# Chris10M/Ev2Hands

Measured on AMD Instinct MI355X. Metric: event-windows/sec at B=256 N=2048 (f16x2), higher is better.
Workload: dtype f32 (each f32 operand split into 2 fp16 planes with per-window power-of-two range scaling, 3 plane products per MAC on the f16 MFMA, f32 accumulate); 1 GPU; TEHNet.forward+MANO both hands, B=256/GPU N=2048 C=4 fp32, E-clouds, random-init 342-key checkpoint, synthetic MANO-shaped assets; global_batch=256, points=2048, channels=4, precision=f16x2, forwards_in_flight=1, world_size_seen=1, parallelism=batch-shard x1

## Files before the change

ev2hands_amd/csrc/forward.hip:

```cpp
#include <cstdarg>
#include <cstdio>
#include <cstdlib>
#include <cstring>

#include "common.hpp"
#include "planes.hpp"
#include "ev2hands_hip.h"
#include "side_stream.hpp"
#include "workspace.hpp"

int ev2h_gemm_init();

static thread_local char g_err[512] = "";

void ev2h_set_error(const char* fmt, ...) {
    va_list ap;
    va_start(ap, fmt);
    vsnprintf(g_err, sizeof(g_err), fmt, ap);
    va_end(ap);
}

extern "C" const char* ev2h_last_error(void) { return g_err; }
extern "C" int ev2h_abi_version(void) { return EV2H_ABI_VERSION; }

// ... 107 lines not shown
    do {                          \
        int rc__ = (expr);        \
        if (rc__) return rc__;    \
    } while (0)

struct DenseOpt {
    const float* group_bias = nullptr; int group_rows = 0, ldbias = 0;
    int taps = 1, rows_per_seq = 0;
    int rowmax_rows = 0;
    int skinny = 0;
    int fam = EV2H_FAM_DENSE;
};

static ev2h_gemm_desc dense_desc(const Call& cx, const ev2h_dense& w, const float* X, int ldx, int M, float* Y, int ldy, int relu, const Rng& rg,
                                 const DenseOpt& o = {}) {
    ev2h_gemm_desc d{};
    d.skinny = o.skinny;
    d.x_amax = rg.xa; d.x_amax2 = rg.xa2; d.x_group_rows = rg.xg; d.y_amax = rg.ya; d.y_group_rows = rg.yg;
    d.X = X; d.ldx = ldx; d.W = w.W; d.ldw = w.ldw; d.Y = Y; d.ldy = ldy;
    d.M = M; d.N = w.O; d.K = w.K;
    d.bias = o.group_bias ? o.group_bias : w.b;
    d.bias_group_rows = o.group_rows; d.ldbias = o.ldbias;
    d.relu = relu; d.post_scale = w.post_scale; d.post_shift = w.post_shift;
    d.taps = o.taps; d.rows_per_seq = o.rows_per_seq; d.rowmax_rows = o.rowmax_rows;
    d.precision = cx.fam_prec(o.fam);
    d.Ws = (cx.prec != EV2H_PREC_F32) ? w.Ws : nullptr;
    d.ws_tile_rows = w.ws_tile_rows;
    d.w_unscale = w.w_unscale;
    return d;
}

static int dense(const Call& cx, const ev2h_dense& w, const float* X, int ldx, int M, float* Y, int ldy, int relu, ev2h_stream_t st, const Rng& rg,
                 const DenseOpt& o = {}) {
    const ev2h_gemm_desc d = dense_desc(cx, w, X, ldx, M, Y, ldy, relu, rg, o);
    return ev2h_gemm(&d, st);
}

static int sa_table(int precision, const ev2h_sa_module& m, const float* feat, int ldf, int B, int Npts, float* P1, ev2h_stream_t st,
                    const uint32_t* feat_amax, uint32_t* p1_amax, float* p1_scale, bool chain = true) {
    int c1sum = 0;
    float extra = 0.f;
    for (int i = 0; i < m.nbranch; ++i) {
        c1sum += m.br[i].C1;
        extra = fmaxf(extra, m.br[i].w1x_norm * (float)m.br[i].radius * 1.0000002f);
    }
    ev2h_gemm_desc g{};
    g.X = feat; g.ldx = ldf; g.W = m.W1f; g.ldw = m.kf; g.Y = P1; g.ldy = c1sum;
    g.M = B * Npts; g.N = c1sum; g.K = m.kf; g.bias = m.b1; g.taps = 1;
    g.precision = precision;
    g.w_unscale = m.w1f_unscale;
    if (precision != EV2H_PREC_F32 && m.W1fs) { g.Ws = m.W1fs; g.ws_tile_rows = 128; }
    if (feat_amax) {
        g.x_amax = feat_amax; g.x_group_rows = Npts;
        g.y_amax = p1_amax; g.y_group_rows = Npts;
        g.y_scale = p1_scale; g.y_bound_w = m.w1f_norm; g.y_bound_b = m.b1_max + extra;
        if (precision == EV2H_PREC_F16 && chain) {
            float wmul = 1.f, badd = g.y_bound_b;
            for (int i = 0; i < m.nbranch; ++i) {
                const float iu = 1.000001f / (m.br[i].w2_unscale > 0.f ? m.br[i].w2_unscale : 1.f);
                wmul = fmaxf(wmul, m.br[i].w2_norm * iu);
                badd = fmaxf(badd, (m.br[i].w2_norm * g.y_bound_b + m.br[i].b2_max) * iu);
            }
            g.y_bound_w *= wmul; g.y_bound_b = badd;
        }
    }
    return ev2h_gemm(&g, st);
}

static bool bf16_direct_layer1(int precision, const ev2h_sa_module& m) {
    static const bool table = getenv("EV2H_L1_TABLE") != nullptr;
    return precision != EV2H_PREC_F32 && m.kf == 8 && !table;
}

static int sa_branches(int precision, const char* tag, const ev2h_sa_module& m, const float* pts4, const float* ctr4, int32_t* const* gidx,
                       const int32_t* cnt, int B, int Npts, const float* P1, float* out, int ldo, ev2h_stream_t st, bool ranges,
                       const uint32_t* p1_amax, const float* p1_scale, uint32_t* out_amax, const float* feat = nullptr, int nfeat = 0,
                       const uint32_t* feat_amax = nullptr, float* xyz_out = nullptr, int xyz_ld = 0, int s_off = 0, int s_cnt = 0) {
    int c1sum = 0;
    for (int i = 0; i < m.nbranch; ++i) c1sum += m.br[i].C1;
    int coff1 = 0, coff3 = 0;
    for (int i = 0; i < m.nbranch; ++i) {
        const ev2h_sa_branch& br = m.br[i];
        ev2h_sa_desc d{};
        d.P1 = P1 + coff1; d.ldp = c1sum; d.pts4 = pts4; d.ctr4 = ctr4; d.gidx = gidx[i];
        d.W1x = br.W1x; d.W2 = br.W2; d.b2 = br.b2; d.W3 = br.W3; d.b3 = br.b3;
        d.out = out + coff3; d.ldo = ldo;
        d.B = B; d.Npts = Npts; d.S = m.npoint; d.K = br.K; d.C1 = br.C1; d.C2 = br.C2; d.C3 = br.C3;
        if (s_cnt > 0) { d.S = s_cnt; d.S_total = m.npoint; d.s_off = s_off; }
        d.precision = precision; d.W2s = br.W2s; d.W3s = br.W3s; d.w2_unscale = br.w2_unscale; d.w3_unscale = br.w3_unscale;
        const bool direct = feat && bf16_direct_layer1(precision, m);
        if (direct) {
            d.feat = feat; d.ldf = 8; d.W1f = m.W1f + (size_t)coff1 * m.kf; d.ldw1f = m.kf; d.b1 = m.b1 + coff1; d.nfeat = nfeat;
            d.w1f_unscale = br.w1f_unscale; d.w1x_unscale = br.w1x_unscale;
            if (ranges) { d.feat_amax = feat_amax; d.w1f_norm = m.w1f_norm; d.b1_max = m.b1_max; }
        }
        if (ranges) {
            if (!direct) { d.p1_scale = p1_scale; d.p1_amax = p1_amax; }
            d.out_amax = out_amax;
            d.w1x_norm = br.w1x_norm; d.dmax = (float)br.radius * 1.0000002f ; d.w2_norm = br.w2_norm; d.b2_max = br.b2_max;
        }
        d.cnt = cnt ? cnt + i : nullptr; d.cnt_ld = m.nbranch;
        if (i == 0 && xyz_out) { d.xyz_out = xyz_out; d.xyz_ld = xyz_ld; }
        char t[40];
        snprintf(t, sizeof(t), "%s.%d", tag, i);
        prof_begin(t, st);
        RUN(ev2h_sa_mlp_max(&d, st));
        prof_end(t, st);
        coff1 += br.C1;
        coff3 += br.C3;
    }
    return EV2H_OK;
}

static int sa_module(int precision, const char* tag, const ev2h_sa_module& m, const float* feat, int ldf, const float* pts4, const float* ctr4,
                     int32_t* const* gidx, const int32_t* cnt, int B, int Npts, float* P1, float* out, int ldo, ev2h_stream_t st,
                     const uint32_t* feat_amax, uint32_t* p1_amax, float* p1_scale, uint32_t* out_amax, int nfeat = 0, float* xyz_out = nullptr,
                     int xyz_ld = 0) {
    if (!bf16_direct_layer1(precision, m)) RUN(sa_table(precision, m, feat, ldf, B, Npts, P1, st, feat_amax, p1_amax, p1_scale));
    return sa_branches(precision, tag, m, pts4, ctr4, gidx, cnt, B, Npts, P1, out, ldo, st, feat_amax != nullptr, p1_amax, p1_scale, out_amax,
                       ldf == 8 ? feat : nullptr, nfeat, feat_amax, xyz_out, xyz_ld);
}

}

static int forward_body(const ev2h_weights* w, const ev2h_mano_consts* const* mano, float* xyz_cm, int B, int C, int N, int mhlnes,
                        const int64_t* fps_init, const ev2h_outputs* out, const Call& cx, bool* forked) {
    const Ws& ws = cx.ws;
    const ev2h_stream_t st = cx.st;
    const int R = B * N;
    const int prec = cx.prec;
    const int prec_sa = cx.fam_prec(EV2H_FAM_SA), prec_rows = cx.fam_prec(EV2H_FAM_ROWS), prec_q = cx.fam_prec(EV2H_FAM_QCONV);
    auto rg = [&](int xid, int xg, int yid = -1, int yg = 0, int xid2 = -1) {
        Rng r{};
        if (ws.ranges_on) {
            r.xa = ws.r(xid); r.xg = xg;
            if (xid2 >= 0) r.xa2 = ws.r(xid2);
            if (yid >= 0) { r.ya = ws.r(yid); r.yg = yg; }
        }
        return r;
    };
    if (ws.ranges_on) EV2H_CHECK_HIP(hipMemsetAsync(ws.i(WS_RANGES), 0, ws.L.count[WS_RANGES] * 4, (hipStream_t)st));

    RUN(ev2h_prep_points(xyz_cm, B, C, N, mhlnes, ws.f(WS_PTS4), ws.f(WS_FEAT8), ws.r(R_FEAT), st));
    const bool fork = cx.side != nullptr;
    const ev2h_stream_t sd = fork ? (ev2h_stream_t)cx.side->stream : st;
    RUN(cx.signal_side(EV_INPUT));
    *forked = fork;
    if (!bf16_direct_layer1(prec, w->sa1)) RUN(sa_table(prec_sa, w->sa1, ws.f(WS_FEAT8), 8, B, N, ws.f(WS_P1A), sd, ws.r(R_FEAT), ws.r(R_P1A), ws.p1scale(0)));
    RUN(cx.side_records(EV_SA1_TABLE));
    static const int chunk_env = [] { const char* e = getenv("EV2H_FPS_CHUNKS"); return e ? atoi(e) : -1; }();
    const int chunk_max_wg = chunk_env > 1 ? chunk_env : (N <= 2048 ? 0x7fffffff : 256), chunk_min_b = chunk_env > 1 ? 1 : 8;
    const bool chunked = fork && chunk_env != 0 && B >= chunk_min_b && 3 * B <= chunk_max_wg && bf16_direct_layer1(prec, w->sa1) && w->sa1.npoint % FPS_CHUNKS == 0;
    const bool side_queries = chunked && B >= 64 && N <= 2048;
    int32_t* gi1[3] = {ws.i(WS_GIDX1_0), ws.i(WS_GIDX1_1), ws.i(WS_GIDX1_2)};
    double rad1[3]; int ns1[3];
    for (int i = 0; i < 3; ++i) { rad1[i] = w->sa1.br[i].radius; ns1[i] = w->sa1.br[i].K; }
    const int S[3] = {512, 128, 128};
    const int64_t* init[3] = {fps_init, fps_init + 2 * (size_t)B, fps_init + 3 * (size_t)B};
    int32_t* idx[3] = {ws.i(WS_FPS1), ws.i(WS_FPSM_L), ws.i(WS_FPSM_R)};
    float* ctr[3] = {ws.f(WS_CTR1), ws.f(WS_CTRM_L), ws.f(WS_CTRM_R)};
    static const bool unfused_fp1 = getenv("EV2H_FP1_UNFUSED") != nullptr;
    const bool fp1_fused = prec != EV2H_PREC_F32 && w->fp1m.W1fs && !unfused_fp1;
    auto late_selections = [&](bool with_samplings) -> int {
        if (fp1_fused) {
            RUN(ev2h_three_nn_interp(ws.f(WS_PTS4), ws.f(WS_CTR1), B, N, 512, nullptr, 0, 0, nullptr, 0, ws.i(WS_NN1_IDX), ws.f(WS_NN1_W), nullptr, sd));
            RUN(cx.side_records(EV_FP1_NN));
        }
        if (with_samplings) RUN(ev2h_fps_multi(ws.f(WS_PTS4), B, N, 2, S + 1, init + 1, idx + 1, ctr + 1, sd));
        for (int h = 0; h < 2; ++h) {
            const ev2h_sa_module& m = w->mano_sa1[h];
            double rad[2]; int ns[2];
            int32_t* gi[2] = {ws.i(hand(WS_GIDXM0_L, h)), ws.i(hand(WS_GIDXM1_L, h))};
            for (int i = 0; i < 2; ++i) { rad[i] = m.br[i].radius; ns[i] = m.br[i].K; }
            RUN(ev2h_ball_query(ws.f(WS_PTS4), ws.f(hand(WS_CTRM_L, h)), B, N, 128, 2, rad, ns, gi, ws.i(hand(WS_CNTM_L, h)), sd));
        }
        return cx.side_records(EV_HAND_QUERIES);
    };
    if (!chunked) {
        RUN(ev2h_fps_multi(ws.f(WS_PTS4), B, N, 3, S, init, idx, ctr, st));
    } else {
        const int q = w->sa1.npoint / FPS_CHUNKS;
        for (int c = 0; c < FPS_CHUNKS; ++c) {
            RUN(ev2h_fps_multi_chunk(ws.f(WS_PTS4), B, N, side_queries ? 1 : 3, S, init, idx, ctr, c * q, (c + 1) * q, ws.f(WS_FPS_STATE), sd));
            if (side_queries) RUN(ev2h_ball_query_range(ws.f(WS_PTS4), ws.f(WS_CTR1), B, N, 512, c * q, q, 3, rad1, ns1, gi1, ws.i(WS_CNT1), sd));
            RUN(cx.side_records(EV_SA1_QUARTER0 + c));
        }
    }
    if (!chunked) RUN(cx.signal_side(EV_SAMPLED));
    int32_t* gi2[2] = {ws.i(WS_GIDX2_0), ws.i(WS_GIDX2_1)};
    {
        const ev2h_sa_module& m = w->sa2;
        RUN(ev2h_fps(ws.f(WS_CTR1), B, 512, 128, fps_init + (size_t)B, ws.i(WS_FPS2), ws.f(WS_CTR2), sd));
        double rad[2]; int ns[2];
        for (int i = 0; i < 2; ++i) { rad[i] = m.br[i].radius; ns[i] = m.br[i].K; }
        RUN(ev2h_ball_query(ws.f(WS_CTR1), ws.f(WS_CTR2), B, 512, 128, 2, rad, ns, gi2, ws.i(WS_CNT2), sd));
        RUN(cx.side_records(EV_SA2_QUERY));
    }
    if (!side_queries) RUN(late_selections(false));
    {
        const ev2h_sa_module& m = w->sa1;
        if (!chunked) {
            RUN(ev2h_ball_query(ws.f(WS_PTS4), ws.f(WS_CTR1), B, N, 512, 3, rad1, ns1, gi1, ws.i(WS_CNT1), st));
            RUN(cx.wait_side(EV_SA1_TABLE));
            RUN(sa_branches(prec_sa, "sa1", m, ws.f(WS_PTS4), ws.f(WS_CTR1), gi1, ws.i(WS_CNT1), B, N, ws.f(WS_P1A), ws.f(WS_L1CAT), 576, st, ws.ranges_on,
                            ws.r(R_P1A), ws.p1scale(0), ws.r(R_L1A), ws.f(WS_FEAT8), C, ws.r(R_FEAT)));
        } else {
            const int q = m.npoint / FPS_CHUNKS;
            for (int c = 0; c < FPS_CHUNKS; ++c) {
                RUN(cx.wait_side(EV_SA1_QUARTER0 + c));
                if (!side_queries) RUN(ev2h_ball_query_range(ws.f(WS_PTS4), ws.f(WS_CTR1), B, N, 512, c * q, q, 3, rad1, ns1, gi1, ws.i(WS_CNT1), st));
                RUN(sa_branches(prec_sa, "sa1", m, ws.f(WS_PTS4), ws.f(WS_CTR1), gi1, ws.i(WS_CNT1), B, N, ws.f(WS_P1A), ws.f(WS_L1CAT), 576, st, ws.ranges_on,
                                ws.r(R_P1A), ws.p1scale(0), ws.r(R_L1A), ws.f(WS_FEAT8), C, ws.r(R_FEAT), nullptr, 0, c * q, q));
            }
        }
    }
    {
        const ev2h_sa_module& m = w->sa2;
        RUN(cx.wait_side(EV_SA2_QUERY));
        RUN(sa_module(prec_sa, "sa2", m, ws.f(WS_L1CAT), 576, ws.f(WS_CTR1), ws.f(WS_CTR2), gi2, ws.i(WS_CNT2), B, 512, ws.f(WS_P1B), ws.f(WS_L2BUF), 520, st,
                      ws.r(R_L1A), ws.r(R_P1B), ws.p1scale(1), ws.r(R_L2), 0, ws.f(WS_L2BUF) + 512, 520));
    }
    RUN(dense(cx, w->sa3[0], ws.f(WS_L2BUF), 520, B * 128, ws.f(WS_SA3H1), 256, 1, st, rg(R_L2, 128, R_SA3H1, 128, R_FEAT)));
    RUN(dense(cx, w->sa3[1], ws.f(WS_SA3H1), 256, B * 128, ws.f(WS_SA3H2), 512, 1, st, rg(R_SA3H1, 128, R_SA3H2, 128)));
    RUN(dense(cx, w->sa3[2], ws.f(WS_SA3H2), 512, B * 128, ws.f(WS_L3), 1024, 1, st, rg(R_SA3H2, 128, R_L3, 1), {.rowmax_rows = 128}));
    RUN(dense(cx, w->fp3_bcast, ws.f(WS_L3), 1024, B, ws.f(WS_FP3BIAS), 256, 0, st, rg(R_L3, 1), {.skinny = 1}));
    if (side_queries) {
        RUN(cx.signal_side(EV_ENC_SA3));
        RUN(late_selections(true));
    }
    RUN(dense(cx, w->fp3_skip, ws.f(WS_L2BUF), 520, B * 128, ws.f(WS_FP3H), 256, 1, st, rg(R_L2, 128, R_FP3H, 128, R_FEAT),
              {.group_bias = ws.f(WS_FP3BIAS), .group_rows = 128, .ldbias = 256}));
    RUN(dense(cx, w->fp3_1, ws.f(WS_FP3H), 256, B * 128, ws.f(WS_FP3O), 256, 1, st, rg(R_FP3H, 128, R_FP3O, 128)));
    RUN(ev2h_three_nn_interp(ws.f(WS_CTR1), ws.f(WS_CTR2), B, 512, 128, ws.f(WS_FP3O), 256, 256, ws.f(WS_L1CAT) + 320, 576,
                             ws.i(WS_NN2_IDX), ws.f(WS_NN2_W), ws.r(R_L1B), st));
    RUN(dense(cx, w->fp2[0], ws.f(WS_L1CAT), 576, B * 512, ws.f(WS_FP2H), 256, 1, st, rg(R_L1A, 512, R_FP2H, 512, R_L1B)));
    RUN(dense(cx, w->fp2[1], ws.f(WS_FP2H), 256, B * 512, ws.f(WS_L1NEW), 128, 1, st, rg(R_FP2H, 512, R_L1NEW, 512)));
    static const bool unfused_cls = getenv("EV2H_CLS_UNFUSED") != nullptr;
    static const bool unfused_zsum = getenv("EV2H_ATTN_UNFUSED_ZSUM") != nullptr;
    static const bool l0_f32 = getenv("EV2H_L0_F32") != nullptr;
    const bool cls_fused = prec != EV2H_PREC_F32 && w->clsm.W2s && !unfused_cls;
    const ev2h_gemm_desc qd = dense_desc(cx, w->qconv0, ws.f(WS_L0), 256, R, ws.f(WS_Q1), 512, 1, rg(R_L0, N),
                                         {.taps = 3, .rows_per_seq = N, .fam = EV2H_FAM_QCONV});
    const bool zsum_ok = !unfused_zsum && prec != EV2H_PREC_F32 && w->qconv0.Ws && ev2h_gemm_bf16_zsum_supported(&qd);
    const bool l0_bf16 = prec == EV2H_PREC_BF16 && fp1_fused && cls_fused && zsum_ok && !l0_f32;
    const bool l0_f16 = prec == EV2H_PREC_F16 && prec_rows == EV2H_PREC_F16 && prec_q == EV2H_PREC_F16 && ws.ranges_on && fp1_fused && cls_fused && zsum_ok && !l0_f32;
    const bool l0_16 = l0_bf16 || l0_f16;
    g_last_l0_bf16 = l0_bf16 ? 1 : (l0_f16 ? 2 : 0);
    if (fp1_fused) {
        const ev2h_sa_module& m = w->fp1m;
        RUN(cx.wait_side(EV_FP1_NN));
        RUN(sa_table(prec_rows, m, ws.f(WS_L1NEW), 128, B, 512, ws.f(WS_FP1T), st, ws.r(R_L1NEW), ws.r(R_FP1T), ws.p1scale(4), false));
        ev2h_fp_desc d{};
        d.T = ws.f(WS_FP1T); d.ldt = 128; d.nn_idx = ws.i(WS_NN1_IDX); d.nn_w = ws.f(WS_NN1_W);
        d.b2 = m.br[0].b2; d.b3 = m.br[0].b3; d.W2s = m.br[0].W2s; d.W3s = m.br[0].W3s;
        d.w2_unscale = m.br[0].w2_unscale; d.w3_unscale = m.br[0].w3_unscale;
        d.out = ws.f(WS_L0); d.ldo = 256; d.B = B; d.N = N; d.S = 512; d.C1 = 128; d.C2 = 128; d.C3 = 256; d.precision = prec_rows;
        if (ws.ranges_on) {
            d.t_scale = ws.p1scale(4); d.t_amax = ws.r(R_FP1T); d.w2_norm = m.br[0].w2_norm; d.b2_max = m.br[0].b2_max; d.out_amax = ws.r(R_L0);
        }
        prof_begin("fp1", st);
        RUN(ev2h_fp_mlp_ex(&d, 0, l0_16, st, l0_f16 ? ws.p1scale(5) : nullptr, m.br[0].w3_norm, m.br[0].b3_max));
        prof_end("fp1", st);
    } else {
        RUN(ev2h_three_nn_interp(ws.f(WS_PTS4), ws.f(WS_CTR1), B, N, 512, ws.f(WS_L1NEW), 128, 128, ws.f(WS_FP1IN), 128,
                                 ws.i(WS_NN1_IDX), ws.f(WS_NN1_W), ws.r(R_FP1IN), st));
        RUN(dense(cx, w->fp1[0], ws.f(WS_FP1IN), 128, R, ws.f(WS_FP1H1), 128, 1, st, rg(R_FP1IN, N, R_FP1H1, N)));
        RUN(dense(cx, w->fp1[1], ws.f(WS_FP1H1), 128, R, ws.f(WS_FP1H2), 128, 1, st, rg(R_FP1H1, N, R_FP1H2, N)));
        RUN(dense(cx, w->fp1[2], ws.f(WS_FP1H2), 128, R, ws.f(WS_L0), 256, 1, st, rg(R_FP1H2, N, R_L0, N)));
    }
    RUN(cx.signal_side(EV_L0));
    if (cls_fused) {
        const ev2h_sa_branch& c = w->clsm;
        ev2h_fp_desc d{};
        d.T = ws.f(WS_L0); d.ldt = 256; d.b2 = c.b2; d.b3 = c.b3; d.W2s = c.W2s; d.W3s = c.W3s;
        d.w2_unscale = c.w2_unscale; d.w3_unscale = c.w3_unscale;
        d.out = ws.f(WS_LOGITS_PM); d.ldo = 4; d.out_cols = 4; d.no_relu_out = 1; d.out_cm = out->class_logits; d.out_cm_stride = out->logits_stride;
        d.B = B; d.N = N; d.C1 = c.C1; d.C2 = c.C2; d.C3 = c.C3; d.precision = prec_rows;
        if (ws.ranges_on) { d.t_amax = ws.r(R_L0); d.w2_norm = c.w2_norm; d.b2_max = c.b2_max; }
        RUN(ev2h_fp_mlp_ex(&d, l0_16, 0, sd, l0_f16 ? ws.p1scale(5) : nullptr));
    } else {
        RUN(dense(cx, w->cls0, ws.f(WS_L0), 256, R, ws.f(WS_CLSH), 256, 1, sd, rg(R_L0, N, R_CLSH, N)));
        RUN(dense(cx, w->cls4, ws.f(WS_CLSH), 256, R, ws.f(WS_LOGITS_PM), 4, 0, sd, rg(R_CLSH, N)));
        RUN(ev2h_transpose_logits(ws.f(WS_LOGITS_PM), B, N, out->class_logits, out->logits_stride, sd));
    }
    RUN(cx.side_records(EV_LOGITS));
    if (zsum_ok) {
        RUN(cx.wait_side(EV_LOGITS));
        prof_begin("qconv0", st);
        RUN(ev2h_gemm_bf16_zsum(&qd, ws.f(WS_LOGITS_PM), ws.f(WS_ZPART), l0_16, st, l0_f16 ? ws.p1scale(5) : nullptr));
        prof_end("qconv0", st);
    } else {
        prof_begin("qconv0", st);
        RUN(ev2h_gemm(&qd, st));
        prof_end("qconv0", st);
    }
    RUN(cx.wait_side(EV_LOGITS));
    if (zsum_ok) {
        RUN(ev2h_attn_simfold_partials(ws.f(WS_ZPART), 128, ws.f(WS_LOGITS_PM), B, N, w->qconv4T[0], w->qconv4T[1], w->qconv4[0].b, w->qconv4[1].b,
                                       ws.f(WS_SIM), st));
    } else {
        RUN(ev2h_attn_sim_folded(ws.f(WS_LOGITS_PM), ws.f(WS_Q1), 512, B, N, w->qconv4T[0], w->qconv4T[1], w->qconv4[0].b, w->qconv4[1].b,
                                 ws.f(WS_ZPART), ws.f(WS_SIM), st));
    }
    if (l0_bf16) RUN(ev2h_attn_context_bf16rows(ws.f(WS_SIM), ws.f(WS_L0), 256, B, N, ws.f(WS_HF8), w->l0_unscale, st));
    else if (l0_f16) RUN(ev2h_attn_context_f16rows(ws.f(WS_SIM), ws.f(WS_L0), 256, B, N, ws.f(WS_HF8), ws.r(R_HF), B, w->l0_unscale, ws.p1scale(5), st));
    else RUN(ev2h_attn_context(ws.f(WS_SIM), ws.f(WS_L0), 256, B, N, ws.f(WS_HF8), ws.r(R_HF), B, w->l0_unscale, st));
    RUN(cx.wait_side(EV_HAND_QUERIES));
    RUN(cx.signal_side(EV_HF8));
    for (int h = 0; h < 2; ++h) {
        const ev2h_sa_module& m = w->mano_sa1[h];
        ev2h_stream_t sh = (h == 1) ? sd : st;
        int32_t* gi[2] = {ws.i(hand(WS_GIDXM0_L, h)), ws.i(hand(WS_GIDXM1_L, h))};
        RUN(sa_module(prec_sa, h ? "manoR" : "manoL", m, ws.f(WS_HF8) + (size_t)h * R * 8, 8, ws.f(WS_PTS4), ws.f(hand(WS_CTRM_L, h)), gi, ws.i(hand(WS_CNTM_L, h)), B, N, ws.f(hand(WS_P1M_L, h)), ws.f(hand(WS_M1BUF_L, h)), 520, sh,
                      ws.r(R_HF + h), ws.r(R_P1M + h), ws.p1scale(2 + h), ws.r(R_M1 + h), 4, ws.f(hand(WS_M1BUF_L, h)) + 512, 520));
        RUN(dense(cx, w->mano_sa2[h][0], ws.f(hand(WS_M1BUF_L, h)), 520, B * 128, ws.f(hand(WS_MSA2H_L, h)), 256, 1, sh, rg(R_M1 + h, 128, R_MSA2H + h, 128, R_FEAT)));
        RUN(dense(cx, w->mano_sa2[h][1], ws.f(hand(WS_MSA2H_L, h)), 256, B * 128, ws.f(hand(WS_M2_L, h)), 512, 1, sh, rg(R_MSA2H + h, 128, R_M2 + h, 1), {.rowmax_rows = 128}));
        RUN(dense(cx, w->head0[h], ws.f(hand(WS_M2_L, h)), 512, B, ws.f(hand(WS_FC1_L, h)), 1024, 1, sh, rg(R_M2 + h, 1, R_FC1 + h, 1), {.skinny = 1}));
        const int ldprm = out->params_stride ? (int)out->params_stride : w->head4[h].O;
        RUN(dense(cx, w->head4[h], ws.f(hand(WS_FC1_L, h)), 1024, B, out->params[h], ldprm, 0, sh, rg(R_FC1 + h, 1), {.skinny = 1}));
        if (mano[h]) RUN(ev2h_mano(mano[h], out->params[h], ldprm, B, out->vertices[h], out->vertices_stride, out->joints[h], out->joints_stride, sh));
    }
    return EV2H_OK;
}

extern "C" int ev2h_forward(const ev2h_weights* w, const ev2h_mano_consts* mano_left, const ev2h_mano_consts* mano_right,
                            float* xyz_cm, int B, int C, int N, int mhlnes, const int64_t* fps_init, const ev2h_outputs* out,
                            void* workspace, size_t workspace_bytes, ev2h_stream_t st) {
    EV2H_CHECK_ARG(w && xyz_cm && fps_init && out && workspace);
    EV2H_CHECK_ARG(B > 0 && N >= 128 && N <= 32768 && (C == 4 || C == 5));
    EV2H_CHECK_ARG(out->class_logits && out->params[0] && out->params[1]);
    EV2H_CHECK_ARG(!mano_left || (out->vertices[0] && out->joints[0]));
    EV2H_CHECK_ARG(!mano_right || (out->vertices[1] && out->joints[1]));
    EV2H_CHECK_ARG((out->logits_stride == 0 || out->logits_stride >= (size_t)4 * N) && (out->params_stride == 0 || out->params_stride >= (size_t)w->head4[0].O));
    EV2H_CHECK_ARG(w->head4[0].O == w->head4[1].O && w->head4[0].O >= 17 && w->head4[0].O <= 61);
    for (int h = 0; h < 2; ++h) {
        const ev2h_mano_consts* mc = h ? mano_right : mano_left;
        if (mc && 3 + mc->ncomps + 13 != w->head4[h].O) {
            ev2h_set_error("ev2h_forward: the checkpoint regresses %d pose coefficients per hand, the %s MANO model takes %d", w->head4[h].O - 16,
                           h ? "right" : "left", mc->ncomps);
            return EV2H_ERR_ARG;
        }
    }
    EV2H_CHECK_ARG(out->params_stride <= 0x7fffffff);
    EV2H_CHECK_ARG((out->vertices_stride == 0 || out->vertices_stride >= 2334) && (out->joints_stride == 0 || out->joints_stride >= 63));
    EV2H_CHECK_ARG(w->sa1.npoint == 512 && w->sa2.npoint == 128 && w->mano_sa1[0].npoint == 128 && w->mano_sa1[1].npoint == 128);
    EV2H_CHECK_ARG(w->sa1.nbranch == 3 && w->sa2.nbranch == 2 && w->mano_sa1[0].nbranch == 2 && w->mano_sa1[1].nbranch == 2);
    if ((w->precision == EV2H_PREC_F16X2 || w->precision == EV2H_PREC_F16) && !(w->flags & (EV2H_W_EQUALIZED | EV2H_W_UNEQUALIZED_OK))) {
        ev2h_set_error("ev2h_forward: F16X2 / F16 weights are not channel-equalised (pack them with ev2h_pack_weights(..., EV2H_PACK_EQUALIZE), "
                       "or set EV2H_W_UNEQUALIZED_OK in ev2h_weights.flags to run them anyway, or use BF16X3 / F32)");
        return EV2H_ERR_ARG;
    }
    RUN(ev2h_init());
    Call cx;
    cx.prec = w->precision;
    cx.f16_families = w->precision == EV2H_PREC_F16 ? w->f16_families : 0;
    cx.st = st;
    Ws& ws = cx.ws;
    ws.base = static_cast<char*>(workspace);
    ws.B = B;
    ws.ranges_on = (w->precision == EV2H_PREC_F16X2 || w->precision == EV2H_PREC_F16);
    build_layout(ws.L, B, N);
    if (workspace_bytes < ws.L.total) {
        ev2h_set_error("ev2h_forward: workspace too small (%zu < %zu bytes)", workspace_bytes, ws.L.total);
        return EV2H_ERR_WORKSPACE;
    }
// ... 17 lines not shown
```

ev2hands_amd/csrc/points.hip:

```cpp
#include <cstdlib>
#include "common.hpp"
#include "ev2hands_hip.h"

namespace {

typedef float f32x2 __attribute__((ext_vector_type(2)));

__device__ __forceinline__ float sqnorm3(float x, float y, float z) {
    return __fadd_rn(__fadd_rn(__fmul_rn(x, x), __fmul_rn(y, y)), __fmul_rn(z, z));
}

__global__ __launch_bounds__(256) void prep_points_kernel(float* __restrict__ xyz_cm, int C, int N, int mhlnes,
                                                          float4* __restrict__ pts4, float4* __restrict__ feat8,
                                                          unsigned* __restrict__ amax) {
    const int b = blockIdx.y;
    const int n = blockIdx.x * 256 + threadIdx.x;
    float* base = xyz_cm + (size_t)b * C * N;
    float f[8];
#pragma unroll
    for (int c = 0; c < 8; ++c) f[c] = (c < C && n < N) ? base[(size_t)c * N + n] : 0.f;
    if (mhlnes && n < N) {
        float s = f[3];
        for (int c = 4; c < C; ++c) s = __fadd_rn(s, f[c]);
        s = s / (float)(C - 3);
        f[2] = s;
        base[(size_t)2 * N + n] = s;
    }
    if (amax) {
        unsigned m = 0u;
#pragma unroll
        for (int c = 0; c < 8; ++c) m = max(m, __float_as_uint(f[c]) & 0x7fffffffu);
        m = wave_max_u32_dpp(m);
        if ((threadIdx.x & 63) == 0 && m) atomicMax(&amax[b], m);
    }
    if (n >= N) return;
    pts4[(size_t)b * N + n] = make_float4(f[0], f[1], f[2], sqnorm3(f[0], f[1], f[2]));
    feat8[((size_t)b * N + n) * 2 + 0] = make_float4(f[0], f[1], f[2], f[3]);
    feat8[((size_t)b * N + n) * 2 + 1] = make_float4(f[4], f[5], f[6], f[7]);
}

struct FpsJobs {
    int njobs;
    int S[3];
    const int64_t* init[3];
    int32_t* idx[3];
    float4* ctr[3];
    int s_begin, s_end;
    float* state; int state_ld;
};

template <int PPT, int THREADS = 256, bool LDS_PTS = true>
__global__ __launch_bounds__(THREADS) void fps_kernel(const float4* __restrict__ pts4, int N, FpsJobs jobs) {
    extern __shared__ __attribute__((aligned(16))) char smem_raw[];
    float4* spts = reinterpret_cast<float4*>(smem_raw);
    constexpr int NW = THREADS / 64;
    __shared__ unsigned long long skey[2][NW];

    const int b = blockIdx.x;
    const int job = blockIdx.y;
    const int S = jobs.S[job];
    const int tid = threadIdx.x, lane = tid & 63, wave = tid >> 6;
    const float4* src = pts4 + (size_t)b * N;

    constexpr bool REG_PTS = !(PPT >= 32 && THREADS >= 1024);
    float px[REG_PTS ? PPT : 1], py[REG_PTS ? PPT : 1], pz[REG_PTS ? PPT : 1], md[PPT];
#pragma unroll
    for (int j = 0; j < PPT; ++j) {
        const int p = j * THREADS + tid;
        if constexpr (REG_PTS || LDS_PTS) {
            float4 v = (p < N) ? src[p] : make_float4(0.f, 0.f, 0.f, 0.f);
            if (LDS_PTS && p < N) spts[p] = v;
            if constexpr (REG_PTS) { px[j] = v.x; py[j] = v.y; pz[j] = v.z; }
        }
        md[j] = 1e10f;
    }
    __syncthreads();
    int tid_v = tid;
    auto coord = [&](int j, float& x, float& y, float& z) {
        if constexpr (REG_PTS) { x = px[j]; y = py[j]; z = pz[j]; }
        else {
            const unsigned pc = (unsigned)min(j * THREADS + tid_v, N - 1);
            const float4 v = *reinterpret_cast<const float4*>(reinterpret_cast<const char*>(src) + (size_t)pc * sizeof(float4));
            x = v.x; y = v.y; z = v.z;
        }
    };

    int far = (int)jobs.init[job][b];
    int32_t* oidx = jobs.idx[job] + (size_t)b * S;
    float4* octr = jobs.ctr[job] + (size_t)b * S;
    const int i_begin = min(jobs.s_begin, S), i_end = min(jobs.s_end, S);
    if (i_begin >= i_end) return;
    float* st = jobs.state ? jobs.state + ((size_t)b * jobs.njobs + job) * jobs.state_ld : nullptr;
    if (i_begin > 0) {
#pragma unroll
        for (int j = 0; j < PPT; ++j) md[j] = st[j * THREADS + tid];
        far = reinterpret_cast<const int*>(st)[jobs.state_ld - 4];
    }

    for (int i = i_begin; i < i_end; ++i) {
        if constexpr (!REG_PTS) asm volatile("" : "+v"(tid_v));
        const float4 c = LDS_PTS ? spts[far] : src[far];
        if (tid == 0) { oidx[i] = far; octr[i] = c; }
        unsigned long long best = 0ull;
        if constexpr (PPT >= 2) {
            const f32x2 cx = {c.x, c.x}, cy = {c.y, c.y}, cz = {c.z, c.z};
#pragma unroll
            for (int j = 0; j < PPT; j += 2) {
                float x0, y0, z0, x1, y1, z1;
                coord(j, x0, y0, z0);
                coord(j + 1, x1, y1, z1);
                const f32x2 dx = f32x2{x0, x1} - cx, dy = f32x2{y0, y1} - cy, dz = f32x2{z0, z1} - cz;
                const f32x2 d = (dx * dx + dy * dy) + dz * dz;
#pragma unroll
                for (int e = 0; e < 2; ++e) {
                    const int p = (j + e) * THREADS + tid;
                    if (d[e] < md[j + e]) md[j + e] = d[e];
                    const unsigned long long key =
                        ((unsigned long long)__float_as_uint(md[j + e]) << 32) | (unsigned long long)(0xffffffffu - (unsigned)p);
                    if (p < N && key > best) best = key;
                }
                if constexpr (!REG_PTS) {
                    if ((j & 6) == 6) __builtin_amdgcn_sched_barrier(0);
                }
            }
        } else {
#pragma unroll
            for (int j = 0; j < PPT; ++j) {
                const int p = j * THREADS + tid;
                float x0, y0, z0;
                coord(j, x0, y0, z0);
                const float dx = __fsub_rn(x0, c.x), dy = __fsub_rn(y0, c.y), dz = __fsub_rn(z0, c.z);
                const float d = sqnorm3(dx, dy, dz);
                if (d < md[j]) md[j] = d;
                const unsigned long long key =
                    ((unsigned long long)__float_as_uint(md[j]) << 32) | (unsigned long long)(0xffffffffu - (unsigned)p);
                if (p < N && key > best) best = key;
            }
        }
        best = wave_max_u64_dpp(best);
        if (lane == 0) skey[i & 1][wave] = best;
        __syncthreads();
        unsigned long long k0 = skey[i & 1][0];
#pragma unroll
        for (int w = 1; w < NW; ++w) { const unsigned long long kw = skey[i & 1][w]; k0 = k0 > kw ? k0 : kw; }
        far = (int)(0xffffffffu - (unsigned)(k0 & 0xffffffffull));
    }
    if (i_end < S) {
#pragma unroll
        for (int j = 0; j < PPT; ++j) st[j * THREADS + tid] = md[j];
        if (tid == 0) reinterpret_cast<int*>(st)[jobs.state_ld - 4] = far;
    }
}

struct BallArgs {
    int nrad;
    float r2[3];
    int K[3];
    int32_t* gidx[3];
    int32_t* cnt;
    int cpw;
    int nchunk;
    int s_off, s_cnt;
};

constexpr int BALL_CTR_PER_WG = 4, BALL_UNR = 4;

__global__ __launch_bounds__(256) void ball_query_kernel(const float4* __restrict__ pts4, const float4* __restrict__ ctr4,
                                                         int N, int S, BallArgs a) {
    const int L = xcd_remap(blockIdx.x, gridDim.x);
    const int b = L / a.nchunk;
    const int tid = threadIdx.x, lane = tid & 63, wave = tid >> 6;
    const float4* src = pts4 + (size_t)b * N;
    (void)tid;
    const int s_begin = a.s_off + (L - b * a.nchunk) * a.cpw;
    const int wave_u = __builtin_amdgcn_readfirstlane(wave);
    for (int s = s_begin + wave_u; s < s_begin + a.cpw && s < a.s_off + a.s_cnt; s += 4) {
        const float4 c = ctr4[(size_t)b * S + s];
        int cnt[3] = {0, 0, 0};
        int first[3] = {0, 0, 0};
        char* gbase[3];
#pragma unroll
        for (int i = 0; i < 3; ++i) gbase[i] = (i < a.nrad) ? reinterpret_cast<char*>(a.gidx[i] + ((size_t)b * S + s) * a.K[i]) : nullptr;
        auto step = [&](int base, auto tail) -> bool {
            constexpr bool TAIL = decltype(tail)::value;
            float d[BALL_UNR];
#pragma unroll
            for (int u = 0; u < BALL_UNR; ++u) {
                const int p = base + 64 * u + lane;
                const unsigned off = (unsigned)(TAIL ? (p < N ? p : N - 1) : p) * (unsigned)sizeof(float4);
                const float4 q = *reinterpret_cast<const float4*>(reinterpret_cast<const char*>(src) + off);
                const float dot = __fmaf_rn(c.z, q.z, __fmaf_rn(c.y, q.y, __fmul_rn(c.x, q.x)));
                d[u] = __fadd_rn(__fadd_rn(__fmul_rn(-2.f, dot), c.w), q.w);
            }
            bool done = true;
#pragma unroll
            for (int i = 0; i < 3; ++i) {
                if (i < a.nrad && cnt[i] < a.K[i]) {
#pragma unroll
                    for (int u = 0; u < BALL_UNR; ++u) {
                        const int p = base + 64 * u + lane;
                        const bool in = (!TAIL || p < N) && !(d[u] > a.r2[i]);
                        const unsigned long long m = __builtin_amdgcn_ballot_w64(in);
                        if (m != 0ull) {
                            if (cnt[i] == 0) first[i] = base + 64 * u + __ffsll((long long)m) - 1;
                            const int pos = (int)__builtin_amdgcn_mbcnt_hi((unsigned)(m >> 32), __builtin_amdgcn_mbcnt_lo((unsigned)m, (unsigned)cnt[i]));
                            if (in && pos < a.K[i]) *reinterpret_cast<int32_t*>(gbase[i] + (unsigned)pos * 4u) = p;
                            cnt[i] += __popcll(m);
                        }
                    }
                    done = done && (cnt[i] >= a.K[i]);
                }
            }
            return done;
        };
        for (int base = 0; base < N; base += 64 * BALL_UNR) {
            const bool done = (base + 64 * BALL_UNR <= N) ? step(base, std::false_type{}) : step(base, std::true_type{});
            if (done) break;
        }
#pragma unroll
        for (int i = 0; i < 3; ++i) {
            if (i < a.nrad) {
                const int have = cnt[i] < a.K[i] ? cnt[i] : a.K[i];
                for (int pos = have + lane; pos < a.K[i]; pos += 64)
                    a.gidx[i][((size_t)b * S + s) * a.K[i] + pos] = first[i];
                if (a.cnt && lane == 0) a.cnt[((size_t)b * S + s) * a.nrad + i] = have;
            }
        }
    }
}

constexpr int NN_PTS_PER_WG = 256;
constexpr int NN_MAX_N2 = 4096;

__global__ __launch_bounds__(256) void three_nn_interp_kernel(const float4* __restrict__ pts1, const float4* __restrict__ pts2,
                                                              int N1, int N2, const float* __restrict__ feat2, int ldf2, int D,
                                                              float* __restrict__ out, int ldo,
                                                              int32_t* __restrict__ nn_idx, float* __restrict__ nn_w,
                                                              unsigned* __restrict__ amax, int ppw) {
    extern __shared__ __attribute__((aligned(16))) char smem_raw[];
    float4* s2 = reinterpret_cast<float4*>(smem_raw);
    int* sidx = reinterpret_cast<int*>(s2 + N2);
    float* sw = reinterpret_cast<float*>(sidx + NN_PTS_PER_WG * 3);
    const int b = blockIdx.y;
    const int tid = threadIdx.x, lane = tid & 63, wave = tid >> 6;
    for (int p = tid; p < N2; p += 256) s2[p] = pts2[(size_t)b * N2 + p];
    __syncthreads();

    const int n = blockIdx.x * ppw + tid;
    if (tid < ppw && n < N1) {
        const float4 q = pts1[(size_t)b * N1 + n];
        float d0 = INFINITY, d1 = INFINITY, d2 = INFINITY;
        int i0 = 0, i1 = 0, i2 = 0;
        for (int s = 0; s < N2; ++s) {
            const float4 c = s2[s];
            const float dot = __fmaf_rn(q.z, c.z, __fmaf_rn(q.y, c.y, __fmul_rn(q.x, c.x)));
            const float d = __fadd_rn(__fadd_rn(__fmul_rn(-2.f, dot), q.w), c.w);
            if (d < d2) {
                if (d < d1) {
                    d2 = d1; i2 = i1;
                    if (d < d0) { d1 = d0; i1 = i0; d0 = d; i0 = s; }
                    else        { d1 = d;  i1 = s; }
                } else { d2 = d; i2 = s; }
            }
        }
        const float r0 = __fdiv_rn(1.0f, __fadd_rn(d0, 1e-8f));
        const float r1 = __fdiv_rn(1.0f, __fadd_rn(d1, 1e-8f));
        const float r2 = __fdiv_rn(1.0f, __fadd_rn(d2, 1e-8f));
        const float norm = __fadd_rn(__fadd_rn(r0, r1), r2);
        const float w0 = __fdiv_rn(r0, norm), w1 = __fdiv_rn(r1, norm), w2 = __fdiv_rn(r2, norm);
        sidx[tid * 3 + 0] = i0; sidx[tid * 3 + 1] = i1; sidx[tid * 3 + 2] = i2;
        sw[tid * 3 + 0] = w0; sw[tid * 3 + 1] = w1; sw[tid * 3 + 2] = w2;
        if (nn_idx) {
            int32_t* o = nn_idx + ((size_t)b * N1 + n) * 3;
            o[0] = i0; o[1] = i1; o[2] = i2;
        }
        if (nn_w) {
            float* o = nn_w + ((size_t)b * N1 + n) * 3;
            o[0] = w0; o[1] = w1; o[2] = w2;
        }
    }
    __syncthreads();
    if (!out) return;
    const int D4 = D >> 2;
    float am = 0.f;
    const int pw = ppw >> 2;
#pragma unroll 1
    for (int t0 = wave * pw; t0 < wave * pw + pw; t0 += 4) {
        if (blockIdx.x * ppw + t0 >= N1) break;
        for (int c = lane; c < D4; c += 64) {
            float4 a[4], bq[4], cq[4];
            float w0[4], w1[4], w2[4];
#pragma unroll
            for (int u = 0; u < 4; ++u) {
                const int t = t0 + u;
                const int j0 = sidx[t * 3 + 0], j1 = sidx[t * 3 + 1], j2 = sidx[t * 3 + 2];
                w0[u] = sw[t * 3 + 0]; w1[u] = sw[t * 3 + 1]; w2[u] = sw[t * 3 + 2];
                const bool live = blockIdx.x * ppw + t < N1;
                a[u] = reinterpret_cast<const float4*>(feat2 + ((size_t)b * N2 + (live ? j0 : 0)) * ldf2)[c];
                bq[u] = reinterpret_cast<const float4*>(feat2 + ((size_t)b * N2 + (live ? j1 : 0)) * ldf2)[c];
                cq[u] = reinterpret_cast<const float4*>(feat2 + ((size_t)b * N2 + (live ? j2 : 0)) * ldf2)[c];
            }
#pragma unroll
// ... 140 lines not shown
```

Measured before the change: 23010 event-windows/s.

## Rework FPS argmax with u32 min-distances and uneven chunk boundaries

The farthest-point-sampling loop now keeps minimum distances as unsigned bit patterns and gives each thread a contiguous block of points. That lets each thread take a 32-bit max, and the 64-bit key is built only once per wave through a ballot and readlane instead of once per point. The cross-wave reduction also uses DPP max plus ballot in place of a serial loop. Separately, the four SA1 chunks are split unevenly (6/8/9/9 of 32) so the main stream can start consuming earlier chunks sooner. The risks are tie-break correctness (the lowest index must still win) and the changed state layout that is saved between chunks.

New measurement: 23190 event-windows/s, median of 4. No clear change (+0.8%).

```diff
diff --git a/ev2hands_amd/csrc/forward.hip b/ev2hands_amd/csrc/forward.hip
--- a/ev2hands_amd/csrc/forward.hip
+++ b/ev2hands_amd/csrc/forward.hip
@@ -283,6 +283,11 @@
     const int chunk_max_wg = chunk_env > 1 ? chunk_env : (N <= 2048 ? 0x7fffffff : 256), chunk_min_b = chunk_env > 1 ? 1 : 8;
     const bool chunked = fork && chunk_env != 0 && B >= chunk_min_b && 3 * B <= chunk_max_wg && bf16_direct_layer1(prec, w->sa1) && w->sa1.npoint % FPS_CHUNKS == 0;
     const bool side_queries = chunked && B >= 64 && N <= 2048;
+    static constexpr int UNEVEN32[FPS_CHUNKS + 1] = {0, 6, 14, 23, 32};
+    static_assert(FPS_CHUNKS == 4, "UNEVEN32 lists four chunks");
+    const bool uneven = side_queries && w->sa1.npoint % 32 == 0;
+    int qb[FPS_CHUNKS + 1];
+    for (int c = 0; c <= FPS_CHUNKS; ++c) qb[c] = uneven ? UNEVEN32[c] * (w->sa1.npoint / 32) : c * (w->sa1.npoint / FPS_CHUNKS);
     int32_t* gi1[3] = {ws.i(WS_GIDX1_0), ws.i(WS_GIDX1_1), ws.i(WS_GIDX1_2)};
     double rad1[3]; int ns1[3];
     for (int i = 0; i < 3; ++i) { rad1[i] = w->sa1.br[i].radius; ns1[i] = w->sa1.br[i].K; }
@@ -310,10 +315,9 @@
     if (!chunked) {
         RUN(ev2h_fps_multi(ws.f(WS_PTS4), B, N, 3, S, init, idx, ctr, st));
     } else {
-        const int q = w->sa1.npoint / FPS_CHUNKS;
         for (int c = 0; c < FPS_CHUNKS; ++c) {
-            RUN(ev2h_fps_multi_chunk(ws.f(WS_PTS4), B, N, side_queries ? 1 : 3, S, init, idx, ctr, c * q, (c + 1) * q, ws.f(WS_FPS_STATE), sd));
-            if (side_queries) RUN(ev2h_ball_query_range(ws.f(WS_PTS4), ws.f(WS_CTR1), B, N, 512, c * q, q, 3, rad1, ns1, gi1, ws.i(WS_CNT1), sd));
+            RUN(ev2h_fps_multi_chunk(ws.f(WS_PTS4), B, N, side_queries ? 1 : 3, S, init, idx, ctr, qb[c], qb[c + 1], ws.f(WS_FPS_STATE), sd));
+            if (side_queries) RUN(ev2h_ball_query_range(ws.f(WS_PTS4), ws.f(WS_CTR1), B, N, 512, qb[c], qb[c + 1] - qb[c], 3, rad1, ns1, gi1, ws.i(WS_CNT1), sd));
             RUN(cx.side_records(EV_SA1_QUARTER0 + c));
         }
     }
@@ -336,12 +340,12 @@
             RUN(sa_branches(prec_sa, "sa1", m, ws.f(WS_PTS4), ws.f(WS_CTR1), gi1, ws.i(WS_CNT1), B, N, ws.f(WS_P1A), ws.f(WS_L1CAT), 576, st, ws.ranges_on,
                             ws.r(R_P1A), ws.p1scale(0), ws.r(R_L1A), ws.f(WS_FEAT8), C, ws.r(R_FEAT)));
         } else {
-            const int q = m.npoint / FPS_CHUNKS;
             for (int c = 0; c < FPS_CHUNKS; ++c) {
+                const int q = qb[c + 1] - qb[c];
                 RUN(cx.wait_side(EV_SA1_QUARTER0 + c));
-                if (!side_queries) RUN(ev2h_ball_query_range(ws.f(WS_PTS4), ws.f(WS_CTR1), B, N, 512, c * q, q, 3, rad1, ns1, gi1, ws.i(WS_CNT1), st));
+                if (!side_queries) RUN(ev2h_ball_query_range(ws.f(WS_PTS4), ws.f(WS_CTR1), B, N, 512, qb[c], q, 3, rad1, ns1, gi1, ws.i(WS_CNT1), st));
                 RUN(sa_branches(prec_sa, "sa1", m, ws.f(WS_PTS4), ws.f(WS_CTR1), gi1, ws.i(WS_CNT1), B, N, ws.f(WS_P1A), ws.f(WS_L1CAT), 576, st, ws.ranges_on,
-                                ws.r(R_P1A), ws.p1scale(0), ws.r(R_L1A), ws.f(WS_FEAT8), C, ws.r(R_FEAT), nullptr, 0, c * q, q));
+                                ws.r(R_P1A), ws.p1scale(0), ws.r(R_L1A), ws.f(WS_FEAT8), C, ws.r(R_FEAT), nullptr, 0, qb[c], q));
             }
         }
     }
diff --git a/ev2hands_amd/csrc/points.hip b/ev2hands_amd/csrc/points.hip
--- a/ev2hands_amd/csrc/points.hip
+++ b/ev2hands_amd/csrc/points.hip
@@ -63,16 +63,21 @@
     const float4* src = pts4 + (size_t)b * N;
 
     constexpr bool REG_PTS = !(PPT >= 32 && THREADS >= 1024);
-    float px[REG_PTS ? PPT : 1], py[REG_PTS ? PPT : 1], pz[REG_PTS ? PPT : 1], md[PPT];
+    constexpr bool CONTIG = REG_PTS;
+    auto pidx = [&](int j) { return CONTIG ? tid * PPT + j : j * THREADS + tid; };
+    constexpr unsigned FPS_PAST_END = 0u, FPS_MD_INIT = 0x501502f9u;
+    static_assert(__builtin_bit_cast(unsigned, 1e10f) == FPS_MD_INIT, "bit pattern of the reference's initial minimum");
+    float px[REG_PTS ? PPT : 1], py[REG_PTS ? PPT : 1], pz[REG_PTS ? PPT : 1];
+    unsigned md[PPT];
 #pragma unroll
     for (int j = 0; j < PPT; ++j) {
-        const int p = j * THREADS + tid;
+        const int p = pidx(j);
         if constexpr (REG_PTS || LDS_PTS) {
             float4 v = (p < N) ? src[p] : make_float4(0.f, 0.f, 0.f, 0.f);
             if (LDS_PTS && p < N) spts[p] = v;
             if constexpr (REG_PTS) { px[j] = v.x; py[j] = v.y; pz[j] = v.z; }
         }
-        md[j] = 1e10f;
+        md[j] = p < N ? FPS_MD_INIT : FPS_PAST_END;
     }
     __syncthreads();
     int tid_v = tid;
@@ -93,7 +98,7 @@
     float* st = jobs.state ? jobs.state + ((size_t)b * jobs.njobs + job) * jobs.state_ld : nullptr;
     if (i_begin > 0) {
 #pragma unroll
-        for (int j = 0; j < PPT; ++j) md[j] = st[j * THREADS + tid];
+        for (int j = 0; j < PPT; ++j) md[j] = reinterpret_cast<const unsigned*>(st)[pidx(j)];
         far = reinterpret_cast<const int*>(st)[jobs.state_ld - 4];
     }
 
@@ -101,7 +106,6 @@
         if constexpr (!REG_PTS) asm volatile("" : "+v"(tid_v));
         const float4 c = LDS_PTS ? spts[far] : src[far];
         if (tid == 0) { oidx[i] = far; octr[i] = c; }
-        unsigned long long best = 0ull;
         if constexpr (PPT >= 2) {
             const f32x2 cx = {c.x, c.x}, cy = {c.y, c.y}, cz = {c.z, c.z};
 #pragma unroll
@@ -111,43 +115,56 @@
                 coord(j + 1, x1, y1, z1);
                 const f32x2 dx = f32x2{x0, x1} - cx, dy = f32x2{y0, y1} - cy, dz = f32x2{z0, z1} - cz;
                 const f32x2 d = (dx * dx + dy * dy) + dz * dz;
-#pragma unroll
-                for (int e = 0; e < 2; ++e) {
-                    const int p = (j + e) * THREADS + tid;
-                    if (d[e] < md[j + e]) md[j + e] = d[e];
-                    const unsigned long long key =
-                        ((unsigned long long)__float_as_uint(md[j + e]) << 32) | (unsigned long long)(0xffffffffu - (unsigned)p);
-                    if (p < N && key > best) best = key;
-                }
+                md[j] = min(md[j], __float_as_uint(d[0]));
+                md[j + 1] = min(md[j + 1], __float_as_uint(d[1]));
                 if constexpr (!REG_PTS) {
                     if ((j & 6) == 6) __builtin_amdgcn_sched_barrier(0);
                 }
             }
         } else {
-#pragma unroll
-            for (int j = 0; j < PPT; ++j) {
-                const int p = j * THREADS + tid;
-                float x0, y0, z0;
-                coord(j, x0, y0, z0);
-                const float dx = __fsub_rn(x0, c.x), dy = __fsub_rn(y0, c.y), dz = __fsub_rn(z0, c.z);
-                const float d = sqnorm3(dx, dy, dz);
-                if (d < md[j]) md[j] = d;
-                const unsigned long long key =
-                    ((unsigned long long)__float_as_uint(md[j]) << 32) | (unsigned long long)(0xffffffffu - (unsigned)p);
-                if (p < N && key > best) best = key;
-            }
-        }
-        best = wave_max_u64_dpp(best);
-        if (lane == 0) skey[i & 1][wave] = best;
+            float x0, y0, z0;
+            coord(0, x0, y0, z0);
+            const float dx = __fsub_rn(x0, c.x), dy = __fsub_rn(y0, c.y), dz = __fsub_rn(z0, c.z);
+            md[0] = min(md[0], __float_as_uint(sqnorm3(dx, dy, dz)));
+        }
+        unsigned m = md[0];
+#pragma unroll
+        for (int j = 1; j < PPT; ++j) m = max(m, md[j]);
+        int jb = PPT - 1;
+#pragma unroll
+        for (int j = PPT - 2; j >= 0; --j) jb = md[j] == m ? j : jb;
+        const int pb = pidx(jb);
+        const unsigned wm = wave_max_u32_dpp(m);
+        unsigned wlo;
+        if constexpr (CONTIG) {
+            const int first = __builtin_ctzll(__ballot(m == wm));
+            wlo = ~(unsigned)__builtin_amdgcn_readlane(pb, first);
+        } else {
+            wlo = wave_max_u32_dpp(m == wm ? ~(unsigned)pb : 0u);
+        }
+        if (lane == 0) skey[i & 1][wave] = ((unsigned long long)wm << 32) | wlo;
         __syncthreads();
-        unsigned long long k0 = skey[i & 1][0];
-#pragma unroll
-        for (int w = 1; w < NW; ++w) { const unsigned long long kw = skey[i & 1][w]; k0 = k0 > kw ? k0 : kw; }
-        far = (int)(0xffffffffu - (unsigned)(k0 & 0xffffffffull));
+        if constexpr (CONTIG) {
+            const unsigned long long kw = skey[i & 1][lane & (NW - 1)];
+            const unsigned hi = (unsigned)(kw >> 32);
+            unsigned gm = hi;
+#define EV2H_DPP_MAX(ctrl) gm = max(gm, (unsigned)__builtin_amdgcn_update_dpp(0, (int)gm, ctrl, 0xf, 0xf, false))
+            EV2H_DPP_MAX(0xb1);
+            EV2H_DPP_MAX(0x4e);
+            if constexpr (NW >= 8) EV2H_DPP_MAX(0x141);
+            if constexpr (NW >= 16) EV2H_DPP_MAX(0x140);
+#undef EV2H_DPP_MAX
+            far = (int)~(unsigned)__builtin_amdgcn_readlane((int)(unsigned)kw, __builtin_ctzll(__ballot(hi == gm)));
+        } else {
+            unsigned long long k0 = skey[i & 1][0];
+#pragma unroll
+            for (int w = 1; w < NW; ++w) { const unsigned long long kw = skey[i & 1][w]; k0 = k0 > kw ? k0 : kw; }
+            far = (int)~(unsigned)k0;
+        }
     }
     if (i_end < S) {
 #pragma unroll
-        for (int j = 0; j < PPT; ++j) st[j * THREADS + tid] = md[j];
+        for (int j = 0; j < PPT; ++j) reinterpret_cast<unsigned*>(st)[pidx(j)] = md[j];
         if (tid == 0) reinterpret_cast<int*>(st)[jobs.state_ld - 4] = far;
     }
 }
```
